# jinseokbae/neural_marionette

Measured on AMD Instinct MI355X. Metric: voxel-frames/sec (64^3, T=16), higher is better.
Workload: dtype f32 (conv products as 3x f16-split MFMA with f32 accumulate, fp32-equivalent; everything else f32); 1 GPU; AIST++-shaped synthetic clips 64^3 T=16 B=4/GPU, full NeuralMarionette.forward (detector + 11 losses + HSVRNNBVH.encode, best-of-10), fp32, random-init weights; grid=64, T=16, clips_per_gpu=4, global_clips=4, conv_mode=split16, parallelism=clip-sharded x1 (no data-path collective)

## Files before the change

### neural_marionette_amd/csrc/nm_api.hip

```cpp
#include "nm_ctx.h"
#include <mutex>
#include "nm_grad.h"
#include "nm_up2c.h"
#include <cstdarg>
#include <cstdio>
#include <cstring>
#include <cstdlib>
#include <cmath>
#include <new>
#include <stdexcept>
#include <vector>

static thread_local char g_err[512] = "";

thread_local NmLaunchState* nm_tls_ls = nullptr;
static int env_int(const char* name, int dflt) { const char* e = getenv(name); return e ? atoi(e) : dflt; }
NmLaunchState::NmLaunchState()
    : supertile(env_int("NM355_SUPERTILE", 1)),
      small16(env_int("NM355_SMALL16", 1)),
      ksplit(env_int("NM355_KSPLIT", 1)),
      occ16(env_int("NM355_OCC16", 1)),
      pool16(env_int("NM355_POOL16", 1)),
      f16p2(env_int("NM355_F16P2", 1)),
      f16p(env_int("NM355_F16P", 2)),
// ... 12 lines not shown
      sparse_first(env_int("NM355_SPARSE_FIRST", 1)),
      gn_diag(env_int("NM355_GN_DIAG", 0)),
      lazy_res(env_int("NM355_LAZY_RES", 1)),
      adjust_split(env_int("NM355_ADJUST_SPLIT", 1)),
      hg_core(env_int("NM355_HG_CORE", 1)),
      clip_occ_mfma(env_int("NM355_CLIP_OCC_MFMA", 1)),
      vrnn_chain(env_int("NM355_VRNN_CHAIN", 1)),
      wgrad_k2f16(env_int("NM355_WGRAD_K2F16", 1)),
      convt_f16(env_int("NM355_CONVT_F16", 1)),
      k5_two(env_int("NM355_K5_TWO", 0)),
      clip_late(env_int("NM355_CLIP_LATE", 1)),
      gnb_u8(env_int("NM355_GNB_U8", 1)),
      adj_zwalk(env_int("NM355_ADJ_ZWALK", 1)),
      f16q2(env_int("NM355_F16Q2", 1)),
      vrnn_post_chain(env_int("NM355_VRNN_POST_CHAIN", 2))
      , f16r(env_int("NM355_F16R", 1))
      , up2_mat(env_int("NM355_UP2_MAT", 1))
      , conv_wgs(env_int("NM355_CONV_WGS", 0))
      , fast_decode(env_int("NM355_FAST_DECODE", 1))
      , up2y(env_int("NM355_UP2Y", 1))
      , up2y_march(env_int("NM355_UP2Y_MARCH", 1))
      , up2y_ypad(env_int("NM355_UP2Y_YPAD", 1))
      , up2c_shell(env_int("NM355_UP2C_SHELL", 1))
{ store16_min = env_int("NM355_STORE16_MIN", 32768); chain_spin = env_int("NM355_CHAIN_SPIN", 1 << 20); chain_backoff = env_int("NM355_CHAIN_BACKOFF", 0); chain_drop = env_int("NM355_CHAIN_DROP_WG", 0); chain_stat_delay = env_int("NM355_CHAIN_STAT_DELAY", 0);
  chain_wgpoll = env_int("NM355_CHAIN_WGPOLL", 1);
  chain_xcd_nogo = env_int("NM355_CHAIN_XCD_NOGO", 0);
  chain_xcd = env_int("NM355_CHAIN_XCD", 1); }
NmLaunchState& nm_ls() {
    static thread_local NmLaunchState outside;
    return nm_tls_ls ? *nm_tls_ls : outside;
}

void nm_set_error(const char* fmt, ...) {
    va_list ap; va_start(ap, fmt);
    vsnprintf(g_err, sizeof(g_err), fmt, ap);
    va_end(ap);
}

int nm_abi_catch(const char* fn) noexcept {
    try { throw; }
    catch (const std::bad_alloc&) { nm_set_error("%s: out of host memory (std::bad_alloc)", fn); }
    catch (const std::exception& e) { nm_set_error("%s: internal error: %s", fn, e.what()); }
    catch (...) { nm_set_error("%s: internal error (unknown C++ exception)", fn); }
    return NM_ERR_INTERNAL;
}

// ... 104 lines not shown
    if (hipMalloc(reinterpret_cast<void**>(&c->nf_flag), sizeof(unsigned)) != hipSuccess || hipMemset(c->nf_flag, 0, sizeof(unsigned)) != hipSuccess) {
        nm_set_error("ctx_create: could not allocate the status word");
        delete c;
        return NM_ERR_HIP;
    }
    if (hipHostMalloc(reinterpret_cast<void**>(&c->nf_host), 4 * sizeof(unsigned), hipHostMallocDefault) != hipSuccess) {
        nm_set_error("ctx_create: could not allocate the pinned status slots");
        delete c;
        return NM_ERR_HIP;
    }
    for (int i = 0; i < 4; ++i) c->nf_host[i] = 0;
    { const char* e = getenv("NM355_RANGE_CHECK"); c->range_check = e ? atoi(e) : 1; }
    if (acquire_side_streams(cfg->device, &c->stream2, &c->stream3, &c->side_shared) != hipSuccess ||
        hipEventCreateWithFlags(&c->ev_w[0], hipEventDisableTiming) != hipSuccess ||
        hipEventCreateWithFlags(&c->ev_w[1], hipEventDisableTiming) != hipSuccess ||
        hipEventCreateWithFlags(&c->ev_w[2], hipEventDisableTiming) != hipSuccess ||
        hipEventCreateWithFlags(&c->ev_dy, hipEventDisableTiming) != hipSuccess ||
        hipEventCreateWithFlags(&c->ev_wjoin, hipEventDisableTiming) != hipSuccess ||
        hipEventCreateWithFlags(&c->ev_k5, hipEventDisableTiming) != hipSuccess ||
        hipEventCreateWithFlags(&c->ev_fork, hipEventDisableTiming) != hipSuccess ||
        hipEventCreateWithFlags(&c->ev_clip, hipEventDisableTiming) != hipSuccess ||
        hipEventCreateWithFlags(&c->ev_kp, hipEventDisableTiming) != hipSuccess ||
        hipEventCreateWithFlags(&c->ev_side, hipEventDisableTiming) != hipSuccess ||
        hipEventCreateWithFlags(&c->ev_nf[0], hipEventDisableTiming) != hipSuccess ||
        hipEventCreateWithFlags(&c->ev_nf[1], hipEventDisableTiming) != hipSuccess ||
        hipEventCreateWithFlags(&c->ev_nf[2], hipEventDisableTiming) != hipSuccess ||
        hipEventCreateWithFlags(&c->ev_nf[3], hipEventDisableTiming) != hipSuccess) {
        nm_set_error("ctx_create: could not create the side stream / events");
        if (c->stream2 || c->stream3) release_side_streams(cfg->device, c->stream2, c->stream3, c->side_shared);
        delete c;
        return NM_ERR_HIP;
    }
    *out = c;
    return NM_OK;
} catch (...) { return nm_abi_catch("nm_ctx_create"); }

int nm_ctx_destroy(nm_ctx* ctx) try {
    if (!ctx) return NM_OK;
    (void)hipSetDevice(ctx->cfg.device);
    (void)hipDeviceSynchronize();
    for (void* p : ctx->owned) (void)hipFree(p);
    if (ctx->ws.base) (void)hipFree(ctx->ws.base);
    if (ctx->ws2.base) (void)hipFree(ctx->ws2.base);
    if (ctx->ws_t.base) (void)hipFree(ctx->ws_t.base);
    if (ctx->copy_table) (void)hipFree(ctx->copy_table);
    if (ctx->pack_table) (void)hipFree(ctx->pack_table);
    if (ctx->nf_flag) (void)hipFree(ctx->nf_flag);
    if (ctx->nf_host) (void)hipHostFree(ctx->nf_host);
    for (hipEvent_t e : ctx->ev_nf) if (e) (void)hipEventDestroy(e);
    if (ctx->vrnn.parents) (void)hipFree(ctx->vrnn.parents);
    nm_vrnn_free_graphs(ctx);
    nm_net_free_tape(ctx);
    nm_vrnn_free_tape(ctx);
    if (ctx->stream2 || ctx->stream3) release_side_streams(ctx->cfg.device, ctx->stream2, ctx->stream3, ctx->side_shared);
    if (ctx->wside) (void)hipFree(ctx->wside);
    for (hipEvent_t e : {ctx->ev_fork, ctx->ev_clip, ctx->ev_kp, ctx->ev_side, ctx->ev_w[0], ctx->ev_w[1], ctx->ev_w[2], ctx->ev_dy, ctx->ev_wjoin, ctx->ev_k5}) if (e) (void)hipEventDestroy(e);
    for (const NmProfRec& r : ctx->ls.prof) { (void)hipEventDestroy(r.a); (void)hipEventDestroy(r.b); }
    for (hipEvent_t e : ctx->ls.event_pool) (void)hipEventDestroy(e);
    delete ctx;
    return NM_OK;
} catch (...) { return nm_abi_catch("nm_ctx_destroy"); }

int nm_ctx_set_stream(nm_ctx* ctx, void* hip_stream) try { NmScope nm_scope_(ctx);
    if (!ctx) { nm_set_error("set_stream: null ctx"); return NM_ERR_ARG; }
    hipStream_t ns = static_cast<hipStream_t>(hip_stream);
    if (ns != ctx->stream && ctx->stream_bound) {
        (void)hipSetDevice(ctx->cfg.device);
        int rc = nm_check_hip(hipEventRecord(ctx->ev_fork, ctx->stream), "set_stream: record on the old stream");
        if (!rc) rc = nm_check_hip(hipStreamWaitEvent(ns, ctx->ev_fork, 0), "set_stream: new stream waits for the old one");
        if (!rc) rc = nm_check_hip(hipEventRecord(ctx->ev_fork, ctx->stream2), "set_stream: record on the side stream");
        if (!rc) rc = nm_check_hip(hipStreamWaitEvent(ns, ctx->ev_fork, 0), "set_stream: new stream waits for the side stream");
        if (rc) return rc;
    }
    ctx->stream = ns;
    ctx->stream_bound = true;
    return NM_OK;
} catch (...) { return nm_abi_catch("nm_ctx_set_stream"); }

int nm_ctx_check_nonfinite(nm_ctx* ctx) try { NmScope nm_scope_(ctx);
// ... 358 lines not shown
```

### neural_marionette_amd/csrc/nm_common.h

```cpp
#pragma once
#include <hip/hip_runtime.h>
#include <stdint.h>
#include <vector>

#define NM_OK 0
#define NM_ERR_ARG (-1)
#define NM_ERR_HIP (-2)
#define NM_ERR_STATE (-3)
#define NM_ERR_UNSUPPORTED (-4)
#define NM_ERR_RANGE (-5)
#define NM_ERR_INTERNAL (-6)

typedef float f32x4 __attribute__((ext_vector_type(4)));
typedef float f32x16 __attribute__((ext_vector_type(16)));
typedef _Float16 nm_half8 __attribute__((ext_vector_type(8)));
template <bool SINGLE>
__device__ __forceinline__ f32x16 nm_mfma_lo(nm_half8 a, nm_half8 b, f32x16 c) {
    if constexpr (SINGLE) return c;
    else return __builtin_amdgcn_mfma_f32_32x32x16_f16(a, b, c, 0, 0, 0);
}


typedef unsigned nm_u32x2 __attribute__((ext_vector_type(2)));
typedef __bf16 nm_bf16x2 __attribute__((ext_vector_type(2)));
// ... 93 lines not shown
    if (e != hipSuccess) return nm_check_hip(e, what);
    once.mark();
    return NM_OK;
}
int nm_num_cus();
int nm_abi_catch(const char* fn) noexcept;

struct NmProfRec { hipEvent_t a, b; int variant; double flops; };
struct NmLaunchState {
    int conv_mode = 1;
    bool f16p_all = false;
    bool single = false;
    bool store16 = false;
    int op_in_h = 0, op_out_h = 0;
    int store16_min = 32768;
    int chain_spin = 1 << 20, chain_backoff = 0, chain_drop = 0, chain_fits = -1, post_chain_fits = -1, chain_stat_delay = 0, chain_wgpoll = 1, chain_xcd_nogo = 0, chain_xcd = 1, chain_cus = 0;
    bool prof_on = false;
    hipStream_t prof_stream = nullptr;
    bool prof_all = false;
    double prof_min_flops = 0.0;
    std::vector<NmProfRec> prof;
    std::vector<hipEvent_t> event_pool;
    unsigned* nf_flag = nullptr;
    int supertile, small16, ksplit, occ16, pool16, f16p2, f16p, pool_q, occ_flags, gnb_apply4, defer_sums, wgrad_async, wgrad_wgs, wgrad_tr, tail_rank1, up2c, vrnn_mid, vrnn_gemm, vrnn_graph, sparse_first, gn_diag, lazy_res, adjust_split, hg_core, clip_occ_mfma, vrnn_chain, wgrad_k2f16, convt_f16, k5_two, clip_late, gnb_u8, adj_zwalk, f16q2, vrnn_post_chain, f16r, up2_mat, conv_wgs, fast_decode, up2y, up2y_march, up2y_ypad, up2c_shell;
    NmLaunchState();
};
NmLaunchState& nm_ls();

size_t nm_packed_weight_floats(int ks, int Cin_pad, int Co_pad);
int nm_launch_pack_conv_weight(const float* w_oidhw, int Cout, int Cin, int ks, float* packed,
                               int Cin_pad, int Co_pad, hipStream_t s);
int nm_conv_blocks_per_frame(const ConvGeom& g, int Cin = 16 );
int nm_launch_conv(const TensorRef& in, const float* w_packed, const float* bias, float* out,
                   const ConvGeom& g, float* part , hipStream_t s,
                   int cin_real = 0 ,
                   const void* w_packed16 = nullptr ,
                   int out_h = 0 );
void nm_conv_set_mode(int mode);
int nm_conv_get_mode();
int nm_conv_single();
int nm_launch_pack_conv_weight16(const float* w_oidhw, int Cout, int Cin, int ks, void* packed, int Co_pad, hipStream_t s);
struct NmPackJob {
    const float* src; float* wp; void* wp16;
    int Cout, Cin, ks, Cin_pad, Co_pad, src_cin, flip, blk0, nblk;
    int src_rows;
};
int nm_pack_job_blocks(const NmPackJob& j);
int nm_launch_pack_jobs(const NmPackJob* device_jobs, int njobs, int total_blocks, hipStream_t s);
int nm_occ_blocks_per_frame(int G);
int nm_launch_pack_occ_weight(const float* w_oidhw, int Cout, float* tmp, float* packed, int Co_pad, hipStream_t s);
int nm_launch_conv_k5occ(const float* occ, int N, int G, const float* w_packed, const float* field, float* out, int Cout,
                         int Co_pad, float* part, hipStream_t s, unsigned char* brickmap = nullptr, const float* field_part = nullptr,
                         unsigned char* flags = nullptr ,
                         int out_h = 0 );
bool nm_conv_pool16_eligible(int Cin, int OD, int OH, int OW, bool have_w16);
void nm_conv_prof_enable(int on, hipStream_t stream);
int nm_conv_prof_collect(int variant, double* ms_total, double* flops_total, long long* launches);
void nm_conv_prof_reset();
struct NmProfScope {
    bool on = false; NmProfRec rec{}; hipStream_t s = nullptr;
// ... 27 lines not shown
```

### neural_marionette_amd/csrc/nm_conv.hip

```cpp
#include "nm_common.h"
#include "nm_up2c.h"
#include <type_traits>
#include <utility>
#include <vector>

namespace {

#define NM_SPLIT_SCALE 2048.0f

struct ConvParams {
    const float* in; const float* in_scale; const float* in_shift; float in_slope;
    int N, ID, IH, IW, Cin;
    const float* w; const float* bias;
    float* out; float* part;
    int OD, OH, OW, Cout, Co_pad;
    int ks, stride, pad;
    int bz_l2, by_l2, bx_l2;
    int nbz, nby, nbx;
    int KC;
    int cin_real;
    int up2;
    int HZ, HY, HX, HV, HVp;
    int CVp;
    int ZP;
// ... 2991 lines not shown
    const int io = (p.in_h ? 1 : 0) | (p.out_h ? 2 : 0);
    if (io && (!SINGLE || p.Cin > 128 || p.in2 || p.in_map || !(io & 1))) return io16_unsupported("conv_pool_f16q", p);
    NmProfScope prof(s, conv_flops(p, 8.0), 8);
    if (io) {
        if constexpr (SINGLE) {
            if (io == 3) hipLaunchKernelGGL((conv_pool_f16q_kernel<NT, true, false, 3>), grid, dim3(256), 0, s, p);
            else hipLaunchKernelGGL((conv_pool_f16q_kernel<NT, true, false, 1>), grid, dim3(256), 0, s, p);
        }
    } else
    if (nm_ls().pool_q && p.Cin <= 128) {
        if (p.in2) hipLaunchKernelGGL((conv_pool_f16q_kernel<NT, SINGLE, true>), grid, dim3(256), 0, s, p);
        else hipLaunchKernelGGL((conv_pool_f16q_kernel<NT, SINGLE, false>), grid, dim3(256), 0, s, p);
    } else
    hipLaunchKernelGGL((conv_pool_f16s_kernel<NT, SINGLE>), grid, dim3(256), 0, s, p);
    return nm_check_hip(hipGetLastError(), "conv_pool_f16s launch");
}
template <int NT>
int launch_pool_f16s(const ConvParams& p, dim3 grid, hipStream_t s) {
    return nm_ls().single ? launch_pool_f16s_impl<NT, true>(p, grid, s) : launch_pool_f16s_impl<NT, false>(p, grid, s);
}

template <auto KERNEL>
int launch_persistent(const char* what_attr, const char* what_launch, int variant, bool super_tile, const ConvParams& p_in,
                      size_t lds_bytes, int work_items, hipStream_t s) {
    static NmDeviceOnce attr_set;
    if (int rc = nm_raise_lds_limit(attr_set, 160 * 1024, what_attr, KERNEL)) return rc;
    const int cus = nm_num_cus();
    if (!cus) return NM_ERR_HIP;
    ConvParams p = p_in;
    dim3 grid((unsigned)min(work_items, nm_ls().conv_wgs > 0 ? min(nm_ls().conv_wgs, cus) : cus));
    if (super_tile) choose_super_tile(p, (int)grid.x, p.OD / 4, p.OH / 8, p.OW / 8);
    NmProfScope prof(s, conv_flops(p, 27.0), variant);
    hipLaunchKernelGGL(KERNEL, grid, dim3(512), lds_bytes, s, p);
    return nm_check_hip(hipGetLastError(), what_launch);
}

template <bool SINGLE, int IO = 0>
int launch_f16p_impl(const ConvParams& p, int work_items, hipStream_t s) {
    const size_t lds_bytes = (size_t)8 * 600 * 16 + (size_t)3 * 9 * 4 * 32 * 16 + (size_t)(256 + p.Cout) * sizeof(float);
    return launch_persistent<&conv_f16p_kernel<SINGLE, IO>>("hipFuncSetAttribute(conv_f16p)", "conv_f16p launch", 7, p.Cout == 32, p, lds_bytes, work_items, s);
}
int launch_f16p(const ConvParams& p, int work_items, hipStream_t s) {
    const int io = (p.in_h ? 1 : 0) | (p.out_h ? 2 : 0);
    if (io) {
        if (io != 3 || !nm_ls().single) return io16_unsupported("conv_f16p", p);
        return launch_f16p_impl<true, 3>(p, work_items, s);
    }
    return nm_ls().single ? launch_f16p_impl<true>(p, work_items, s) : launch_f16p_impl<false>(p, work_items, s);
}

template <bool SINGLE, int IO = 0>
int launch_f16p2_impl(const ConvParams& p, int work_items, hipStream_t s) {
    const size_t lds_bytes = (size_t)8 * 600 * 16 + (size_t)2 * 9 * 4 * 64 * 16 + (size_t)(512 + p.Cout) * sizeof(float);
    return launch_persistent<&conv_f16p2_kernel<SINGLE, IO>>("hipFuncSetAttribute(conv_f16p2)", "conv_f16p2 launch", 9, p.Cout == 64, p, lds_bytes, work_items, s);
}
template <int IO>
int launch_f16q2_impl(const ConvParams& p, int work_items, hipStream_t s) {
    const size_t lds_bytes = (size_t)4 * 600 * 16 + (size_t)2 * 27 * 2 * 64 * 16 + (size_t)(512 + p.Cout) * sizeof(float);
    if (lds_bytes > 160 * 1024) { nm_set_error("conv_f16q2: %d output channels exceed the LDS budget", p.Cout); return NM_ERR_UNSUPPORTED; }
    return launch_persistent<&conv_f16q2_kernel<IO>>("hipFuncSetAttribute(conv_f16q2)", "conv_f16q2 launch", 14, p.Cout == 64, p, lds_bytes, work_items, s);
}
template <int IO, int C16T>
int launch_f16r_impl(const ConvParams& p, int work_items, hipStream_t s) {
    const size_t lds_bytes = (size_t)4 * 600 * 16 + (size_t)27 * C16T * 64 * 16 + (size_t)(512 + 32) * sizeof(float) + 2048 + 256 + 1024;
    return launch_persistent<&conv_f16r_kernel<IO, C16T>>("hipFuncSetAttribute(conv_f16r)", "conv_f16r launch", 15, true, p, lds_bytes, work_items, s);
}
int launch_f16p2(const ConvParams& p, int work_items, hipStream_t s) {
    const int io = (p.in_h ? 1 : 0) | (p.out_h ? 2 : 0);
    if (nm_ls().single && nm_ls().f16q2 && (io == 0 || io == 3) && p.Cout <= 1024) {
        return io ? launch_f16q2_impl<3>(p, work_items, s) : launch_f16q2_impl<0>(p, work_items, s);
    }
    if (io) {
        if (io != 3 || !nm_ls().single) return io16_unsupported("conv_f16p2", p);
        return launch_f16p2_impl<true, 3>(p, work_items, s);
    }
    if (nm_ls().single) return launch_f16p2_impl<true>(p, work_items, s);
    return launch_f16p2_impl<false>(p, work_items, s);
}

#ifdef NM_DIAG
unsigned long long* g_stamps = nullptr;
#endif

}

#ifdef NM_DIAG
extern "C" void nm_diag_set_stamps(void* p) { g_stamps = static_cast<unsigned long long*>(p); }
#endif
void nm_conv_set_mode(int mode) { NmLaunchState& l = nm_ls(); l.conv_mode = mode ? 1 : 0; l.f16p_all = mode == 2; l.single = mode == 3 || mode == 4; l.store16 = mode == 4; }
int nm_conv_get_mode() { const NmLaunchState& l = nm_ls(); return l.conv_mode && l.single ? (l.store16 ? 4 : 3) : (l.conv_mode && l.f16p_all ? 2 : l.conv_mode); }
int nm_conv_single() { return nm_ls().conv_mode && nm_ls().single; }

int nm_launch_pack_conv_weight16(const float* w, int Cout, int Cin, int ks, void* packed, int Co_pad, hipStream_t s) {
    if (Co_pad % 32 || Cout > Co_pad) { nm_set_error("pack_conv_weight16: bad padding Cout=%d/%d", Cout, Co_pad); return NM_ERR_ARG; }
    size_t total = (size_t)ks * ks * ks * ((Cin + 15) / 16) * 2 * Co_pad * 8;
    int blocks = (int)min((total + 255) / 256, (size_t)2048);
    hipLaunchKernelGGL(pack_conv_weight16_kernel, dim3(blocks), dim3(256), 0, s, w, Cout, Cin, ks, reinterpret_cast<_Float16*>(packed), Co_pad);
    return nm_check_hip(hipGetLastError(), "pack_conv_weight16 launch");
}

// ... 106 lines not shown
NmProfScope::~NmProfScope() {
    if (!on) return;
    (void)hipEventRecord(rec.b, s);
    nm_ls().prof.push_back(rec);
}

int nm_num_cus() {
    static int cus = 0;
    if (cus == 0) {
        int dev = 0; hipDeviceProp_t prop;
        if (hipGetDevice(&dev) != hipSuccess || hipGetDeviceProperties(&prop, dev) != hipSuccess) { (void)nm_check_hip(hipErrorUnknown, "device query"); return 0; }
        cus = prop.multiProcessorCount > 0 ? prop.multiProcessorCount : 256;
    }
    return cus;
}

void nm_conv_prof_reset() {
    NmLaunchState& l = nm_ls();
    for (const NmProfRec& r : l.prof) { l.event_pool.push_back(r.a); l.event_pool.push_back(r.b); }
    l.prof.clear();
}

int nm_launch_conv(const TensorRef& in, const float* w_packed, const float* bias, float* out,
                   const ConvGeom& g, float* part, hipStream_t s, int cin_real, const void* w_packed16, int out_h) {
    if (in.C % 8 != 0 || g.Co_pad % 32 != 0 || g.Cout > g.Co_pad || g.Cout <= 0) {
        nm_set_error("conv: unsupported channels Cin=%d Cout=%d Co_pad=%d", in.C, g.Cout, g.Co_pad);
        return NM_ERR_ARG;
    }
    const int us = g.up2 ? 2 : 1;
    if ((us * in.D + 2 * g.pad - g.ks) / g.stride + 1 != g.OD || (us * in.H + 2 * g.pad - g.ks) / g.stride + 1 != g.OH ||
        (us * in.W + 2 * g.pad - g.ks) / g.stride + 1 != g.OW) {
        nm_set_error("conv: geometry mismatch in=(%d,%d,%d) k=%d s=%d p=%d out=(%d,%d,%d)", in.D, in.H, in.W,
                     g.ks, g.stride, g.pad, g.OD, g.OH, g.OW);
        return NM_ERR_ARG;
    }
    if ((in.scale == nullptr) != (in.shift == nullptr)) { nm_set_error("conv: scale/shift must come together"); return NM_ERR_ARG; }
    if ((in.brickmap || in.p2) && g.up2) { nm_set_error("conv: a brick-sparse input tensor can only feed the k2 s2 split-fp16 pool kernel"); return NM_ERR_ARG; }
    if (use_up2c(g, in.C)) {
        double flops = 2.0 * in.N * (double)g.OD * g.OH * g.OW * g.Cout * (double)(cin_real > 0 ? cin_real : in.C) * 27.0;
        if (nm_up2y_active()) flops *= 0.5;
        NmProfScope prof(s, flops, 12);
        return nm_launch_conv_up2c(in, g.up2c, bias, out, g.Cout, g.Co_pad, part, s, out_h);
    }
    Tiling t = choose_tiling(g, in.C);
    if (t.lds_bytes > 160 * 1024) { nm_set_error("conv: LDS tile %zu B too large", t.lds_bytes); return NM_ERR_UNSUPPORTED; }
    ConvParams p;
    p.in = in.p; p.in_scale = in.scale; p.in_shift = in.shift; p.in_slope = in.slope;
// ... 19 lines not shown
    p.w16 = (nm_ls().conv_mode == 1 && nm_ls().small16 && w_packed16 && in.C % 8 == 0 && !g.up2 && t.MT == 1 && (t.KC % 16 == 0 || t.KC == in.C)) ? w_packed16 : nullptr;
    if (p.w16) t.lds_bytes = max(t.lds_bytes, (size_t)(((t.KC + 15) & ~15) / 4) * (t.HVp + t.CVp) * 16);
    p.ksplit = 1;
    if (p.w16 && nm_ls().ksplit) {
        const int top = ((min(g.OD, 1 << t.bz_l2) - 1) << (t.bx_l2 + t.by_l2)) + ((min(g.OH, 1 << t.by_l2) - 1) << t.bx_l2) + min(g.OW, 1 << t.bx_l2) - 1;
        const int rw = top / 32 + 1;
        p.ksplit = rw == 1 ? 4 : (rw == 2 ? 2 : 1);
        if (p.ksplit > 1) t.lds_bytes = max(t.lds_bytes, (size_t)4 * t.NT * 16 * 64 * sizeof(float));
    }
#ifdef NM_DIAG
    p.stamps = g_stamps;
#endif
    p.KC = t.KC; p.HZ = t.HZ; p.HY = t.HY; p.HX = t.HX; p.HV = t.HV; p.HVp = t.HVp; p.CVp = t.CVp; p.ZP = t.HY * t.HX;
    dim3 grid((unsigned)(in.N * t.nbz * t.nby * t.nbx), (unsigned)(g.Co_pad / (t.NT * 32)));
    if (pool16_case(t, in.C, w_packed16 != nullptr) && g.ks == 2 && g.stride == 2 && g.pad == 0 && !g.up2) {
        p.w = static_cast<const float*>(w_packed16);
        return t.NT == 2 ? launch_pool_f16s<2>(p, grid, s) : launch_pool_f16s<1>(p, grid, s);
    }
    const bool k3_bricks = w_packed16 && in.C % 16 == 0 && g.ks == 3 && g.stride == 1 && g.pad == 1 && !g.up2 &&
                           g.OD % 4 == 0 && g.OH % 8 == 0 && g.OW % 8 == 0 && g.OD >= 16;
    if (nm_ls().conv_mode == 1 && nm_ls().f16p2 && k3_bricks && g.Cout % 64 == 0) {
        const int work = in.N * (g.OD / 4) * (g.OH / 8) * (g.OW / 8) * (g.Cout / 64);
        p.w = static_cast<const float*>(w_packed16);
        return launch_f16p2(p, work, s);
    }
    if (nm_ls().conv_mode == 1 && nm_ls().single && nm_ls().f16r && nm_ls().f16p && k3_bricks && (in.C == 32 || in.C == 64) && g.Cout == 32 &&
        (p.in_h != 0) == (p.out_h != 0)) {
        const int work = in.N * (g.OD / 4) * (g.OH / 8) * (g.OW / 8);
        p.w = static_cast<const float*>(w_packed16);
        if (in.C == 32) return p.in_h ? launch_f16r_impl<3, 2>(p, work, s) : launch_f16r_impl<0, 2>(p, work, s);
        return p.in_h ? launch_f16r_impl<3, 4>(p, work, s) : launch_f16r_impl<0, 4>(p, work, s);
    }
    if (nm_ls().conv_mode == 1 && nm_ls().f16p && k3_bricks && g.Cout % 32 == 0 && (nm_ls().f16p == 1 || nm_ls().f16p_all || g.Cout == 32)) {
        const int work = in.N * (g.OD / 4) * (g.OH / 8) * (g.OW / 8) * (g.Cout / 32);
        p.w = static_cast<const float*>(w_packed16);
        return launch_f16p(p, work, s);
    }
    if (nm_ls().conv_mode == 1 && w_packed16 && in.C % 16 == 0 && t.MT == 2 && t.bx_l2 == 3 && t.by_l2 == 3 && t.bz_l2 == 2 &&
        g.stride == 1 && (g.ks == 1 || g.ks == 3) && t.HZ == g.ks + 3 && t.HY * t.HX * 2 <= 256) {
        Tiling t16 = t;
        const int area = t.HY * t.HX;
        p.ZP = area + ((4 - (area & 15)) & 15);
        const int hv = t.HZ * p.ZP;
        p.HVp = hv + ((2 - (hv & 7)) & 7);
        const bool blds = (t.NT == 1 && g.ks == 3);
        const size_t bbytes = blds ? (size_t)2 * 9 * 4 * 32 * 16 : 0;
        t16.lds_bytes = max(blds ? (size_t)4 * p.HVp * 16 + bbytes : (size_t)4 * (p.HVp + t.CVp) * 16, (size_t)4 * 64 * 2 * sizeof(float));
        if (t16.lds_bytes <= 80 * 1024) {
            p.w = static_cast<const float*>(w_packed16);
            if (g.ks == 3 && g.up2) return t.NT == 2 ? launch_f16s<2, 2, 3, true>(p, t16, grid, s) : launch_f16s<2, 1, 3, true>(p, t16, grid, s);
            if (g.ks == 3) return t.NT == 2 ? launch_f16s<2, 2, 3, false>(p, t16, grid, s) : launch_f16s<2, 1, 3, false>(p, t16, grid, s);
            if (!g.up2) return t.NT == 2 ? launch_f16s<2, 2, 1, false>(p, t16, grid, s) : launch_f16s<2, 1, 1, false>(p, t16, grid, s);
        }
        p.HVp = t.HVp;
    }
    if (p.in_h || p.out_h) return io16_unsupported("conv (fp32 MFMA kernel)", p);
    if (t.MT == 2 && t.NT == 2) return launch_t<2, 2>(p, t, grid, s);
    if (t.MT == 2 && t.NT == 1) return launch_t<2, 1>(p, t, grid, s);
    if (t.MT == 1 && t.NT == 2) return launch_t<1, 2>(p, t, grid, s);
// ... 49 lines not shown
```

### neural_marionette_amd/csrc/nm_ctx.h

```cpp
#pragma once
#include "nm_common.h"
#include "../../include/nm355.h"
#include <map>
#include <string>
#include <vector>

struct Arena {
    char* base = nullptr;
    size_t cap = 0, top = 0, peak = 0;
    bool dry = false;
    bool overflow = false;

    void* alloc_bytes(size_t bytes) {
        size_t a = (top + 255) & ~(size_t)255;
        top = a + bytes;
        if (top > peak) peak = top;
        if (dry) return reinterpret_cast<void*>((uintptr_t)256);
        if (top > cap) { overflow = true; return nullptr; }
        return base + a;
    }
    float* f(size_t n) { return static_cast<float*>(alloc_bytes(n * sizeof(float))); }
    size_t mark() const { return top; }
    void release(size_t m) { top = m; }
};
// ... 42 lines not shown

struct VrnnW {
    LinearW post0, post2, prior0, prior2, root0, root2, joint0, joint2;
    float *w_ih = nullptr, *w_hh = nullptr, *b_ih = nullptr, *b_hh = nullptr;
    float* h0 = nullptr;
    float* offset_param = nullptr;
    int32_t* parents = nullptr;
    int32_t* order = nullptr;
    int32_t* lvl_joint = nullptr;
    int32_t* lvl_start = nullptr;
    int nlevels = 0;
    std::vector<int32_t> parents_h, order_h;
    bool has_tree = false;
    uint64_t tree_epoch = 0;
};

struct nm_ctx {
    nm_config cfg;
    NmLaunchState ls;
    hipStream_t stream = nullptr;
    bool stream_bound = false;
    hipStream_t stream2 = nullptr;
    hipEvent_t ev_fork = nullptr, ev_clip = nullptr, ev_kp = nullptr, ev_side = nullptr;
    hipStream_t stream3 = nullptr;
    bool side_shared = false;
    hipEvent_t ev_w[3] = {nullptr, nullptr, nullptr}, ev_dy = nullptr, ev_wjoin = nullptr, ev_k5 = nullptr;
    float* wside = nullptr; size_t wside_floats = 0;
    size_t wside_slot = 0, wside_scratch = 0, wside_sc = 0;
    hipEvent_t ev_user_decoder = nullptr;
    unsigned* nf_flag = nullptr;
    unsigned* nf_host = nullptr;
    hipEvent_t ev_nf[4] = {nullptr, nullptr, nullptr, nullptr};
    bool nf_busy[4] = {false, false, false, false};
    uint64_t nf_seq[4] = {0, 0, 0, 0};
    const char* nf_who[4] = {nullptr, nullptr, nullptr, nullptr};
    uint64_t nf_calls = 0;
    unsigned nf_last = 0;
    int range_check = 1;
    int learn_sigma = 0;
    int gauss_cat = 0;
    int affinity_ver = 3;
    int graph_loss_ver = 1;
    int const_intensity = 3;
    int graph_flags = 0;
    bool graph_none() const { return (graph_flags & NM_GRAPH_NONE) != 0; }
    int64_t affinity_numel() const {
// ... 45 lines not shown
```

### neural_marionette_amd/csrc/nm_net.hip

```cpp
#include "nm_ctx.h"
#include "nm_heads.h"
#include "nm_grad.h"
#include "nm_heads_bwd.h"
#include "nm_up2c.h"
#include "nm_hgcore.h"
#include <cmath>
#include <cstdio>
#include <vector>
#include <algorithm>
#include <functional>

struct ConvRec {
    const ConvW* w = nullptr; const NormW* gn = nullptr;
    TensorRef in{}, out{};
    TensorRef upmat{};
    const float* fpart = nullptr; int nblk = 0;
    const double* chsum = nullptr;
    int stride = 1, pad = 0; bool up2 = false;
};
struct ResRec { ConvRec c1, c2, cs; bool has_skip = false; };
struct UpRec { const UpW* w = nullptr; TensorRef in{}, out{}; const float* fpart = nullptr; int nblk = 0; const double* chsum = nullptr; };
struct HgRec { ResRec s1, e1, s2, e2, s3, e3, d3, d2, d1; ConvRec p1, p2, p3; UpRec u3, u2, u1; };
struct FeatRec {
    const FeatNetW* w = nullptr; const float* occ = nullptr; int N = 0, G = 0;
// ... 228 lines not shown
        if (!r && !c->training && nm_conv_get_mode() == 1 && nm_ls().occ16 && nm_ls().sparse_first) {
            const int nblk = nm_occ_blocks_per_frame(G);
            f.field_part = nm_ctx_weight_alloc(c, (size_t)nblk * Cout * 2);
            float* scratch = nm_ctx_weight_alloc(c, G3 * Cout);
            if (!f.field_part || !scratch) r = NM_ERR_HIP;
            else r = nm_launch_conv_k5occ(zero, 1, G, f.occ_w, f.field, scratch, Cout, f.c0.Co_pad, f.field_part, c->stream);
        }
        if (r && !rc) rc = r;
    }
    LinearW linear(const std::string& p, int out, int in) {
        LinearW l; l.in = in; l.out = out; l.w = copy(p + ".weight", (int64_t)out * in); l.b = copy(p + ".bias", out); return l;
    }
};

__global__ void pack_small_kernel(const float* a, int na, const float* b, int nb, float* out) {
    int i = threadIdx.x;
    if (i < na) out[i] = a[i];
    else if (i < na + nb) out[i] = b[i - na];
}

struct Net {
    nm_ctx* c; hipStream_t s; Arena& ws; int rc = NM_OK;
    bool keep = false;
    explicit Net(nm_ctx* ctx) : c(ctx), s(ctx->stream), ws(ctx->ws) {}
    Net(nm_ctx* ctx, hipStream_t stream) : c(ctx), s(stream), ws(ctx->ws) {}
    void release(size_t m) { if (!keep) ws.release(m); }
    bool ok() const { return rc == NM_OK; }
    bool live() const { return rc == NM_OK && !ws.dry; }
    void run(int r) { if (r && !rc) rc = r; }
    float* alloc(size_t n) {
        float* p = ws.f(n);
        if (!p && !rc) { nm_set_error("workspace overflow (needed > %zu bytes)", ws.cap); rc = NM_ERR_STATE; }
        return p;
    }
    int h16(size_t voxels_per_frame) const { return keep && nm_ls().store16 && voxels_per_frame >= (size_t)nm_ls().store16_min ? 1 : 0; }
    float* alloc_e(size_t elems, int h) { return alloc(h ? (elems + 1) / 2 : elems); }
};

TensorRef mk(const float* p, int N, int D, int H, int W, int C, const float* sc = nullptr, const float* sh = nullptr, float slope = 1.0f) {
    TensorRef t; t.p = p; t.scale = sc; t.shift = sh; t.slope = slope; t.N = N; t.D = D; t.H = H; t.W = W; t.C = C; return t;
}
TensorRef with_h(TensorRef t, int h) { t.h = h; return t; }
size_t vox(const TensorRef& t) { return (size_t)t.D * t.H * t.W; }

TensorRef conv_gn(Net& n, const TensorRef& in, const ConvW& w, const NormW* gn, int stride, int pad, float slope_after,
                  float* out_buf = nullptr, bool up2 = false, ConvRec* rec = nullptr) {
    ConvGeom g; g.ks = w.ks; g.stride = stride; g.pad = pad; g.up2 = up2 ? 1 : 0;
    const int us = up2 ? 2 : 1;
    g.OD = (us * in.D + 2 * pad - w.ks) / stride + 1; g.OH = (us * in.H + 2 * pad - w.ks) / stride + 1; g.OW = (us * in.W + 2 * pad - w.ks) / stride + 1;
// ... 1 lines not shown
    const size_t ov = (size_t)g.OD * g.OH * g.OW;
    const int oh = out_buf ? 0 : n.h16(ov);
    TensorRef src = in;
    const bool mat = up2 && rec && n.keep && !out_buf && nm_ls().single && nm_ls().up2_mat && nm_ls().f16r && w.wp16 && w.ks == 3 && stride == 1 && pad == 1 &&
                     w.Cout == 32 && (in.C == 32 || in.C == 64) && g.OD % 4 == 0 && g.OH % 8 == 0 && g.OW % 8 == 0 && g.OD >= 16;
    if (mat) {
        float* upb = n.alloc_e((size_t)in.N * ov * in.C, oh);
        if (n.live()) n.run(nm_launch_upsample2(in, upb, n.s, oh));
        src = with_h(mk(upb, in.N, g.OD, g.OH, g.OW, in.C), oh);
        g.up2 = 0; g.up2c = nullptr;
    }
    float* out = out_buf ? out_buf : n.alloc_e((size_t)in.N * ov * w.Cout, oh);
    float *part = nullptr, *scale = nullptr, *shift = nullptr;
    const int nblk = nm_conv_blocks_per_frame(g, in.C);
    double* chsum = nullptr;
    if (gn) {
        part = n.alloc((size_t)in.N * nblk * w.Cout * 2);
        scale = n.alloc((size_t)in.N * w.Cout); shift = n.alloc((size_t)in.N * w.Cout);
        if (rec && nm_gn_finalize_has_chsum(w.Cout, gn->groups)) chsum = reinterpret_cast<double*>(n.alloc((size_t)in.N * w.Cout * 4));
    }
    if (n.live()) {
        if (in.C != w.Cin_pad) { nm_set_error("conv_gn: input has %d channels, layer expects %d", in.C, w.Cin_pad); n.rc = NM_ERR_STATE; }
        else {
            n.run(nm_launch_conv(src, w.wp, w.bias, out, g, part, n.s, w.Cin, w.wp16, oh));
            if (gn) n.run(nm_launch_gn_finalize(part, in.N, nblk, w.Cout, gn->groups, (double)ov * (w.Cout / gn->groups),
                                                gn->gamma, gn->beta, 1e-5f, scale, shift, n.s, chsum));
            if (gn && nm_ls().gn_diag && !oh) n.run(nm_launch_gn_direct(out, in.N, (int)ov, w.Cout, gn->groups, gn->gamma, gn->beta, 1e-5f, scale, shift, n.s, chsum));
        }
    }
    TensorRef o = with_h(mk(out, in.N, g.OD, g.OH, g.OW, w.Cout, scale, shift, slope_after), oh);
    if (rec) { rec->w = &w; rec->gn = gn; rec->in = in; rec->out = o; rec->fpart = part; rec->nblk = nblk; rec->chsum = chsum; rec->stride = stride; rec->pad = pad; rec->up2 = up2; rec->upmat = mat ? src : TensorRef{}; }
    return o;
}

TensorRef add2(Net& n, const TensorRef& a, const TensorRef* b, float* out_buf = nullptr) {
    const int oh = out_buf ? 0 : n.h16(vox(a));
    float* out = out_buf ? out_buf : n.alloc_e((size_t)a.N * vox(a) * a.C, oh);
    if (n.live()) n.run(nm_launch_apply2(a, b, out, n.s, oh));
    return with_h(mk(out, a.N, a.D, a.H, a.W, a.C), oh);
}

TensorRef res(Net& n, const TensorRef& x, const ResW& w, float* out_buf = nullptr, ResRec* rec = nullptr, bool lazy_sum = false) {
    if (lazy_sum && !rec && !out_buf) {
        TensorRef r1 = conv_gn(n, x, w.c1, &w.n1, 1, 1, LRELU);
        TensorRef r2 = conv_gn(n, r1, w.c2, &w.n2, 1, 1, 1.0f);
        TensorRef sk = w.has_skip ? conv_gn(n, x, w.cs, &w.ns, 1, 0, 1.0f) : x;
        TensorRef o = r2;
// ... 74 lines not shown
        if (!n.rc) {
            if (nm_conv_get_mode() != 1) nm_set_error("hourglass core: conv mode %d (the fused launch is split-fp16 arithmetic: mode 1 only)", nm_conv_get_mode());
            else if (a2.D < 2 || a2.D > 6) nm_set_error("hourglass core: level-2 extent %d (the fused launch takes 2 .. 6)", a2.D);
            else if (nm_hg_core_scratch_items(hp) < 0) nm_set_error("hourglass core: %zu bytes of LDS per frame do not fit", nm_hg_core_lds_bytes(hp));
            else nm_set_error("hourglass core: a layer has no split-fp16 weight pack (or the channel counts do not chain)");
            n.rc = NM_ERR_UNSUPPORTED;
        }
        return a2;
    }
    if (eligible) {
        float* d2out = n.alloc((size_t)a2.N * vox(a2) * w.d2.c2.Cout);
        hp.out = d2out;
        if (n.live()) n.run(nm_launch_hg_core(hp, n.s));
        return mk(d2out, a2.N, a2.D, a2.H, a2.W, w.d2.c2.Cout);
    }
    TensorRef x = res(n, a2, w.e2, nullptr, r ? &r->e2 : nullptr);
    TensorRef s3 = res(n, x, w.s3, nullptr, r ? &r->s3 : nullptr);
    x = res(n, pool(n, x, w.p3, r ? &r->p3 : nullptr), w.e3, nullptr, r ? &r->e3 : nullptr);
    x = res(n, x, w.d3, nullptr, r ? &r->d3 : nullptr);
    TensorRef u = up(n, x, w.u3, op3, r ? &r->u3 : nullptr); x = add2(n, u, &s3);
    return res(n, x, w.d2, nullptr, r ? &r->d2 : nullptr);
}

TensorRef hourglass(Net& n, const TensorRef& x0, const HourglassW& w, int Ng, HgRec* r = nullptr) {
    const int op3 = (Ng / 4) % 2, op2 = (Ng / 2) % 2, op1 = Ng % 2;
    TensorRef s1 = res(n, x0, w.s1, nullptr, r ? &r->s1 : nullptr);
    TensorRef x = res(n, pool(n, x0, w.p1, r ? &r->p1 : nullptr), w.e1, nullptr, r ? &r->e1 : nullptr);
    TensorRef s2 = res(n, x, w.s2, nullptr, r ? &r->s2 : nullptr);
    TensorRef a2 = pool(n, x, w.p2, r ? &r->p2 : nullptr);
    x = hourglass_core(n, a2, w, op3, r);
    TensorRef u = up(n, x, w.u2, op2, r ? &r->u2 : nullptr); x = add2(n, u, &s2);
    x = res(n, x, w.d1, nullptr, r ? &r->d1 : nullptr);
    u = up(n, x, w.u1, op1, r ? &r->u1 : nullptr); x = add2(n, u, &s1);
    return x;
}

TensorRef first_layer(Net& n, const float* occ, int N, int G, const FeatNetW& w, FeatRec* rec = nullptr) {
    const int Cout = w.c0.Cout;
    const size_t G3 = (size_t)G * G * G;
    const int oh = rec ? n.h16(G3) : 0;
    float* out = n.alloc_e((size_t)N * G3 * Cout, oh);
    const int nblk = nm_occ_blocks_per_frame(G);
    float* part = n.alloc((size_t)N * nblk * Cout * 2);
    const bool sparse = !rec && w.field_part && nm_conv_get_mode() == 1 && nm_ls().occ16 && nm_ls().sparse_first &&
                        nm_conv_pool16_eligible(Cout, G / 2, G / 2, G / 2, w.p1.c.wp16 != nullptr);
    unsigned char* bmap = sparse ? reinterpret_cast<unsigned char*>(n.alloc(((size_t)N * nblk + 3) / 4)) : nullptr;
    unsigned char* bflags = sparse ? reinterpret_cast<unsigned char*>(n.alloc(((size_t)N * nblk + 3) / 4)) : nullptr;
    float* scale = n.alloc((size_t)N * Cout); float* shift = n.alloc((size_t)N * Cout);
    double* chsum = (rec && nm_gn_finalize_has_chsum(Cout, w.n0.groups)) ? reinterpret_cast<double*>(n.alloc((size_t)N * Cout * 4)) : nullptr;
    if (n.live()) {
        n.run(nm_launch_conv_k5occ(occ, N, G, w.occ_w, w.field, out, Cout, w.c0.Co_pad, part, n.s, bmap, sparse ? w.field_part : nullptr, bflags, oh));
        n.run(nm_launch_gn_finalize(part, N, nblk, Cout, w.n0.groups, (double)G3 * (Cout / w.n0.groups), w.n0.gamma, w.n0.beta,
                                    1e-5f, scale, shift, n.s, chsum));
        if (nm_ls().gn_diag && !sparse && !oh) n.run(nm_launch_gn_direct(out, N, (int)G3, Cout, w.n0.groups, w.n0.gamma, w.n0.beta, 1e-5f, scale, shift, n.s, chsum));
    }
    TensorRef o = with_h(mk(out, N, G, G, G, Cout, scale, shift, LRELU), oh);
// ... 59 lines not shown
                                         Cc, comb, n.s, c->gauss_cat));
            x = mk(comb, nf, g, g, g, Cc);
            x = conv_gn(n, x, d.adjust, nullptr, 1, 0, LRELU, nullptr, false, tape ? &tape->adjust : nullptr);
        }
        x = conv_gn(n, x, d.d1, &d.dn2, 1, 1, LRELU, nullptr, true, tape ? &tape->d1 : nullptr);
        x = conv_gn(n, x, d.d4, &d.dn5, 1, 1, LRELU, nullptr, false, tape ? &tape->d4 : nullptr);
        x = conv_gn(n, x, d.d8, &d.dn9, 1, 1, LRELU, nullptr, true, tape ? &tape->d8 : nullptr);
        x = conv_gn(n, x, d.d11, &d.dn12, 1, 1, LRELU, nullptr, false, tape ? &tape->d11 : nullptr);
        if (n.live())
            n.run(nm_launch_decoder_tail(x, d.d14, first_frames + (size_t)b0 * ff_stride * G3, ff_stride, T,
                                         target ? target + (size_t)f0 * G3 : nullptr,
                                         (target && chamfer) ? keypoints + (size_t)f0 * K * 4 : nullptr, K, G,
                                         recon + (size_t)f0 * G3, tail_part ? tail_part + (size_t)f0 * tb * 3 : nullptr, n.s));
        n.release(m1);
    }
    n.release(m0);
}

int detector_graph(nm_ctx* c, const float* vox_in, int B, int T, int affinity_on, float* keypoints, float* heatmaps,
                   float* first_feature, float* recon, float* affinity, float* losses,
                   const std::function<int()>* after_keypoints = nullptr, TrainTape* tape = nullptr) {
    Net n(c);
    n.keep = tape != nullptr;
    const DetectorW& d = c->det;
    if (c->graph_none()) affinity_on = 0;
    const int K = c->cfg.nkeypoints, G = c->cfg.grid_size, g = G / 4, F = B * T, N = c->cfg.nneighbor;
    const size_t g3 = (size_t)g * g * g, G3 = (size_t)G * G * G;
    const int Kc = d.head.Cout;
    n.ws.release(0);
    float* feat = n.alloc((size_t)F * g3 * FEAT);
    float* clip_head = n.alloc((size_t)B * g3 * Kc);
    float* heat_part = n.alloc((size_t)F * K * g * (2 * g + 2));
    float* heat_mean = n.alloc((size_t)F * K);
    float* clip_part = n.alloc((size_t)B * 5);
    const int tb = nm_tail_blocks(G);
    float* tail_part = n.alloc((size_t)F * tb * 3);
    float* frame_sums = n.alloc((size_t)F * 3);
    float* aff = affinity_on ? (affinity ? affinity : n.alloc((size_t)N * K * K)) : nullptr;

    auto clip_block = [&]() {
        Net n2(c, c->stream2);
        n2.keep = n.keep;
        float* in = n2.alloc((size_t)B * G3);
        float* fclip = n2.alloc((size_t)B * g3 * 2 * FEAT);
        if (n2.live()) n2.run(nm_launch_mean_t(vox_in, B, T, G3, in, n2.s));
        feature_net(n2, in, B, G, d.clip, g, fclip, tape ? &tape->clip : nullptr);
// ... 944 lines not shown
```

Before: 3976 voxel-frames/s.

## Run hourglass skip-branch residual on a side stream with capped conv workgroups

Result: faster. 4044 voxel-frames/s, median of 6 (+1.7%).

```diff
diff --git a/neural_marionette_amd/csrc/nm_api.hip b/neural_marionette_amd/csrc/nm_api.hip
--- a/neural_marionette_amd/csrc/nm_api.hip
+++ b/neural_marionette_amd/csrc/nm_api.hip
@@ -58,6 +58,9 @@
       , up2y_march(env_int("NM355_UP2Y_MARCH", 1))
       , up2y_ypad(env_int("NM355_UP2Y_YPAD", 1))
       , up2c_shell(env_int("NM355_UP2C_SHELL", 1))
+      , enc_sched(env_int("NM355_ENC_SCHED", 1))
+      , enc_s1(env_int("NM355_ENC_S1", 1))
+      , enc_s1_wgs(env_int("NM355_ENC_S1_WGS", -1))
 { store16_min = env_int("NM355_STORE16_MIN", 32768); chain_spin = env_int("NM355_CHAIN_SPIN", 1 << 20); chain_backoff = env_int("NM355_CHAIN_BACKOFF", 0); chain_drop = env_int("NM355_CHAIN_DROP_WG", 0); chain_stat_delay = env_int("NM355_CHAIN_STAT_DELAY", 0);
   chain_wgpoll = env_int("NM355_CHAIN_WGPOLL", 1);
   chain_xcd_nogo = env_int("NM355_CHAIN_XCD_NOGO", 0);
@@ -208,6 +211,8 @@
         hipEventCreateWithFlags(&c->ev_clip, hipEventDisableTiming) != hipSuccess ||
         hipEventCreateWithFlags(&c->ev_kp, hipEventDisableTiming) != hipSuccess ||
         hipEventCreateWithFlags(&c->ev_side, hipEventDisableTiming) != hipSuccess ||
+        hipEventCreateWithFlags(&c->ev_s1_fork, hipEventDisableTiming) != hipSuccess ||
+        hipEventCreateWithFlags(&c->ev_s1_join, hipEventDisableTiming) != hipSuccess ||
         hipEventCreateWithFlags(&c->ev_nf[0], hipEventDisableTiming) != hipSuccess ||
         hipEventCreateWithFlags(&c->ev_nf[1], hipEventDisableTiming) != hipSuccess ||
         hipEventCreateWithFlags(&c->ev_nf[2], hipEventDisableTiming) != hipSuccess ||
@@ -240,7 +245,7 @@
     nm_vrnn_free_tape(ctx);
     if (ctx->stream2 || ctx->stream3) release_side_streams(ctx->cfg.device, ctx->stream2, ctx->stream3, ctx->side_shared);
     if (ctx->wside) (void)hipFree(ctx->wside);
-    for (hipEvent_t e : {ctx->ev_fork, ctx->ev_clip, ctx->ev_kp, ctx->ev_side, ctx->ev_w[0], ctx->ev_w[1], ctx->ev_w[2], ctx->ev_dy, ctx->ev_wjoin, ctx->ev_k5}) if (e) (void)hipEventDestroy(e);
+    for (hipEvent_t e : {ctx->ev_fork, ctx->ev_clip, ctx->ev_kp, ctx->ev_side, ctx->ev_s1_fork, ctx->ev_s1_join, ctx->ev_w[0], ctx->ev_w[1], ctx->ev_w[2], ctx->ev_dy, ctx->ev_wjoin, ctx->ev_k5}) if (e) (void)hipEventDestroy(e);
     for (const NmProfRec& r : ctx->ls.prof) { (void)hipEventDestroy(r.a); (void)hipEventDestroy(r.b); }
     for (hipEvent_t e : ctx->ls.event_pool) (void)hipEventDestroy(e);
     delete ctx;
diff --git a/neural_marionette_amd/csrc/nm_common.h b/neural_marionette_amd/csrc/nm_common.h
--- a/neural_marionette_amd/csrc/nm_common.h
+++ b/neural_marionette_amd/csrc/nm_common.h
@@ -139,7 +139,7 @@
     std::vector<NmProfRec> prof;
     std::vector<hipEvent_t> event_pool;
     unsigned* nf_flag = nullptr;
-    int supertile, small16, ksplit, occ16, pool16, f16p2, f16p, pool_q, occ_flags, gnb_apply4, defer_sums, wgrad_async, wgrad_wgs, wgrad_tr, tail_rank1, up2c, vrnn_mid, vrnn_gemm, vrnn_graph, sparse_first, gn_diag, lazy_res, adjust_split, hg_core, clip_occ_mfma, vrnn_chain, wgrad_k2f16, convt_f16, k5_two, clip_late, gnb_u8, adj_zwalk, f16q2, vrnn_post_chain, f16r, up2_mat, conv_wgs, fast_decode, up2y, up2y_march, up2y_ypad, up2c_shell;
+    int supertile, small16, ksplit, occ16, pool16, f16p2, f16p, pool_q, occ_flags, gnb_apply4, defer_sums, wgrad_async, wgrad_wgs, wgrad_tr, tail_rank1, up2c, vrnn_mid, vrnn_gemm, vrnn_graph, sparse_first, gn_diag, lazy_res, adjust_split, hg_core, clip_occ_mfma, vrnn_chain, wgrad_k2f16, convt_f16, k5_two, clip_late, gnb_u8, adj_zwalk, f16q2, vrnn_post_chain, f16r, up2_mat, conv_wgs, fast_decode, up2y, up2y_march, up2y_ypad, up2c_shell, enc_sched, enc_s1, enc_s1_wgs;
     NmLaunchState();
 };
 NmLaunchState& nm_ls();
@@ -152,7 +152,8 @@
                    const ConvGeom& g, float* part , hipStream_t s,
                    int cin_real = 0 ,
                    const void* w_packed16 = nullptr ,
-                   int out_h = 0 );
+                   int out_h = 0 ,
+                   int wgs_cap = 0 );
 void nm_conv_set_mode(int mode);
 int nm_conv_get_mode();
 int nm_conv_single();
diff --git a/neural_marionette_amd/csrc/nm_conv.hip b/neural_marionette_amd/csrc/nm_conv.hip
--- a/neural_marionette_amd/csrc/nm_conv.hip
+++ b/neural_marionette_amd/csrc/nm_conv.hip
@@ -3037,13 +3037,15 @@
 
 template <auto KERNEL>
 int launch_persistent(const char* what_attr, const char* what_launch, int variant, bool super_tile, const ConvParams& p_in,
-                      size_t lds_bytes, int work_items, hipStream_t s) {
+                      size_t lds_bytes, int work_items, hipStream_t s, int wgs_cap) {
     static NmDeviceOnce attr_set;
     if (int rc = nm_raise_lds_limit(attr_set, 160 * 1024, what_attr, KERNEL)) return rc;
     const int cus = nm_num_cus();
     if (!cus) return NM_ERR_HIP;
     ConvParams p = p_in;
-    dim3 grid((unsigned)min(work_items, nm_ls().conv_wgs > 0 ? min(nm_ls().conv_wgs, cus) : cus));
+    int wgs = nm_ls().conv_wgs > 0 ? min(nm_ls().conv_wgs, cus) : cus;
+    if (wgs_cap > 0 && wgs_cap < wgs) wgs = min(wgs, max(8, wgs_cap & ~7));
+    dim3 grid((unsigned)min(work_items, wgs));
     if (super_tile) choose_super_tile(p, (int)grid.x, p.OD / 4, p.OH / 8, p.OW / 8);
     NmProfScope prof(s, conv_flops(p, 27.0), variant);
     hipLaunchKernelGGL(KERNEL, grid, dim3(512), lds_bytes, s, p);
@@ -3051,46 +3053,46 @@
 }
 
 template <bool SINGLE, int IO = 0>
-int launch_f16p_impl(const ConvParams& p, int work_items, hipStream_t s) {
+int launch_f16p_impl(const ConvParams& p, int work_items, hipStream_t s, int wgs_cap) {
     const size_t lds_bytes = (size_t)8 * 600 * 16 + (size_t)3 * 9 * 4 * 32 * 16 + (size_t)(256 + p.Cout) * sizeof(float);
-    return launch_persistent<&conv_f16p_kernel<SINGLE, IO>>("hipFuncSetAttribute(conv_f16p)", "conv_f16p launch", 7, p.Cout == 32, p, lds_bytes, work_items, s);
-}
-int launch_f16p(const ConvParams& p, int work_items, hipStream_t s) {
+    return launch_persistent<&conv_f16p_kernel<SINGLE, IO>>("hipFuncSetAttribute(conv_f16p)", "conv_f16p launch", 7, p.Cout == 32, p, lds_bytes, work_items, s, wgs_cap);
+}
+int launch_f16p(const ConvParams& p, int work_items, hipStream_t s, int wgs_cap) {
     const int io = (p.in_h ? 1 : 0) | (p.out_h ? 2 : 0);
     if (io) {
         if (io != 3 || !nm_ls().single) return io16_unsupported("conv_f16p", p);
-        return launch_f16p_impl<true, 3>(p, work_items, s);
-    }
-    return nm_ls().single ? launch_f16p_impl<true>(p, work_items, s) : launch_f16p_impl<false>(p, work_items, s);
+        return launch_f16p_impl<true, 3>(p, work_items, s, wgs_cap);
+    }
+    return nm_ls().single ? launch_f16p_impl<true>(p, work_items, s, wgs_cap) : launch_f16p_impl<false>(p, work_items, s, wgs_cap);
 }
 
 template <bool SINGLE, int IO = 0>
-int launch_f16p2_impl(const ConvParams& p, int work_items, hipStream_t s) {
+int launch_f16p2_impl(const ConvParams& p, int work_items, hipStream_t s, int wgs_cap) {
     const size_t lds_bytes = (size_t)8 * 600 * 16 + (size_t)2 * 9 * 4 * 64 * 16 + (size_t)(512 + p.Cout) * sizeof(float);
-    return launch_persistent<&conv_f16p2_kernel<SINGLE, IO>>("hipFuncSetAttribute(conv_f16p2)", "conv_f16p2 launch", 9, p.Cout == 64, p, lds_bytes, work_items, s);
+    return launch_persistent<&conv_f16p2_kernel<SINGLE, IO>>("hipFuncSetAttribute(conv_f16p2)", "conv_f16p2 launch", 9, p.Cout == 64, p, lds_bytes, work_items, s, wgs_cap);
 }
 template <int IO>
-int launch_f16q2_impl(const ConvParams& p, int work_items, hipStream_t s) {
+int launch_f16q2_impl(const ConvParams& p, int work_items, hipStream_t s, int wgs_cap) {
     const size_t lds_bytes = (size_t)4 * 600 * 16 + (size_t)2 * 27 * 2 * 64 * 16 + (size_t)(512 + p.Cout) * sizeof(float);
     if (lds_bytes > 160 * 1024) { nm_set_error("conv_f16q2: %d output channels exceed the LDS budget", p.Cout); return NM_ERR_UNSUPPORTED; }
-    return launch_persistent<&conv_f16q2_kernel<IO>>("hipFuncSetAttribute(conv_f16q2)", "conv_f16q2 launch", 14, p.Cout == 64, p, lds_bytes, work_items, s);
+    return launch_persistent<&conv_f16q2_kernel<IO>>("hipFuncSetAttribute(conv_f16q2)", "conv_f16q2 launch", 14, p.Cout == 64, p, lds_bytes, work_items, s, wgs_cap);
 }
 template <int IO, int C16T>
-int launch_f16r_impl(const ConvParams& p, int work_items, hipStream_t s) {
+int launch_f16r_impl(const ConvParams& p, int work_items, hipStream_t s, int wgs_cap) {
     const size_t lds_bytes = (size_t)4 * 600 * 16 + (size_t)27 * C16T * 64 * 16 + (size_t)(512 + 32) * sizeof(float) + 2048 + 256 + 1024;
-    return launch_persistent<&conv_f16r_kernel<IO, C16T>>("hipFuncSetAttribute(conv_f16r)", "conv_f16r launch", 15, true, p, lds_bytes, work_items, s);
-}
-int launch_f16p2(const ConvParams& p, int work_items, hipStream_t s) {
+    return launch_persistent<&conv_f16r_kernel<IO, C16T>>("hipFuncSetAttribute(conv_f16r)", "conv_f16r launch", 15, true, p, lds_bytes, work_items, s, wgs_cap);
+}
+int launch_f16p2(const ConvParams& p, int work_items, hipStream_t s, int wgs_cap) {
     const int io = (p.in_h ? 1 : 0) | (p.out_h ? 2 : 0);
     if (nm_ls().single && nm_ls().f16q2 && (io == 0 || io == 3) && p.Cout <= 1024) {
-        return io ? launch_f16q2_impl<3>(p, work_items, s) : launch_f16q2_impl<0>(p, work_items, s);
+        return io ? launch_f16q2_impl<3>(p, work_items, s, wgs_cap) : launch_f16q2_impl<0>(p, work_items, s, wgs_cap);
     }
     if (io) {
         if (io != 3 || !nm_ls().single) return io16_unsupported("conv_f16p2", p);
-        return launch_f16p2_impl<true, 3>(p, work_items, s);
-    }
-    if (nm_ls().single) return launch_f16p2_impl<true>(p, work_items, s);
-    return launch_f16p2_impl<false>(p, work_items, s);
+        return launch_f16p2_impl<true, 3>(p, work_items, s, wgs_cap);
+    }
+    if (nm_ls().single) return launch_f16p2_impl<true>(p, work_items, s, wgs_cap);
+    return launch_f16p2_impl<false>(p, work_items, s, wgs_cap);
 }
 
 #ifdef NM_DIAG
@@ -3243,7 +3245,7 @@
 }
 
 int nm_launch_conv(const TensorRef& in, const float* w_packed, const float* bias, float* out,
-                   const ConvGeom& g, float* part, hipStream_t s, int cin_real, const void* w_packed16, int out_h) {
+                   const ConvGeom& g, float* part, hipStream_t s, int cin_real, const void* w_packed16, int out_h, int wgs_cap) {
     if (in.C % 8 != 0 || g.Co_pad % 32 != 0 || g.Cout > g.Co_pad || g.Cout <= 0) {
         nm_set_error("conv: unsupported channels Cin=%d Cout=%d Co_pad=%d", in.C, g.Cout, g.Co_pad);
         return NM_ERR_ARG;
@@ -3309,19 +3311,19 @@
     if (nm_ls().conv_mode == 1 && nm_ls().f16p2 && k3_bricks && g.Cout % 64 == 0) {
         const int work = in.N * (g.OD / 4) * (g.OH / 8) * (g.OW / 8) * (g.Cout / 64);
         p.w = static_cast<const float*>(w_packed16);
-        return launch_f16p2(p, work, s);
+        return launch_f16p2(p, work, s, wgs_cap);
     }
     if (nm_ls().conv_mode == 1 && nm_ls().single && nm_ls().f16r && nm_ls().f16p && k3_bricks && (in.C == 32 || in.C == 64) && g.Cout == 32 &&
         (p.in_h != 0) == (p.out_h != 0)) {
         const int work = in.N * (g.OD / 4) * (g.OH / 8) * (g.OW / 8);
         p.w = static_cast<const float*>(w_packed16);
-        if (in.C == 32) return p.in_h ? launch_f16r_impl<3, 2>(p, work, s) : launch_f16r_impl<0, 2>(p, work, s);
-        return p.in_h ? launch_f16r_impl<3, 4>(p, work, s) : launch_f16r_impl<0, 4>(p, work, s);
+        if (in.C == 32) return p.in_h ? launch_f16r_impl<3, 2>(p, work, s, wgs_cap) : launch_f16r_impl<0, 2>(p, work, s, wgs_cap);
+        return p.in_h ? launch_f16r_impl<3, 4>(p, work, s, wgs_cap) : launch_f16r_impl<0, 4>(p, work, s, wgs_cap);
     }
     if (nm_ls().conv_mode == 1 && nm_ls().f16p && k3_bricks && g.Cout % 32 == 0 && (nm_ls().f16p == 1 || nm_ls().f16p_all || g.Cout == 32)) {
         const int work = in.N * (g.OD / 4) * (g.OH / 8) * (g.OW / 8) * (g.Cout / 32);
         p.w = static_cast<const float*>(w_packed16);
-        return launch_f16p(p, work, s);
+        return launch_f16p(p, work, s, wgs_cap);
     }
     if (nm_ls().conv_mode == 1 && w_packed16 && in.C % 16 == 0 && t.MT == 2 && t.bx_l2 == 3 && t.by_l2 == 3 && t.bz_l2 == 2 &&
         g.stride == 1 && (g.ks == 1 || g.ks == 3) && t.HZ == g.ks + 3 && t.HY * t.HX * 2 <= 256) {
diff --git a/neural_marionette_amd/csrc/nm_ctx.h b/neural_marionette_amd/csrc/nm_ctx.h
--- a/neural_marionette_amd/csrc/nm_ctx.h
+++ b/neural_marionette_amd/csrc/nm_ctx.h
@@ -88,6 +88,7 @@
     bool stream_bound = false;
     hipStream_t stream2 = nullptr;
     hipEvent_t ev_fork = nullptr, ev_clip = nullptr, ev_kp = nullptr, ev_side = nullptr;
+    hipEvent_t ev_s1_fork = nullptr, ev_s1_join = nullptr;
     hipStream_t stream3 = nullptr;
     bool side_shared = false;
     hipEvent_t ev_w[3] = {nullptr, nullptr, nullptr}, ev_dy = nullptr, ev_wjoin = nullptr, ev_k5 = nullptr;
diff --git a/neural_marionette_amd/csrc/nm_net.hip b/neural_marionette_amd/csrc/nm_net.hip
--- a/neural_marionette_amd/csrc/nm_net.hip
+++ b/neural_marionette_amd/csrc/nm_net.hip
@@ -274,9 +274,12 @@
 struct Net {
     nm_ctx* c; hipStream_t s; Arena& ws; int rc = NM_OK;
     bool keep = false;
+    int conv_wgs = 0;
+    bool s1_fork = false;
+    bool hold = false;
     explicit Net(nm_ctx* ctx) : c(ctx), s(ctx->stream), ws(ctx->ws) {}
     Net(nm_ctx* ctx, hipStream_t stream) : c(ctx), s(stream), ws(ctx->ws) {}
-    void release(size_t m) { if (!keep) ws.release(m); }
+    void release(size_t m) { if (!keep && !hold) ws.release(m); }
     bool ok() const { return rc == NM_OK; }
     bool live() const { return rc == NM_OK && !ws.dry; }
     void run(int r) { if (r && !rc) rc = r; }
@@ -324,7 +327,7 @@
     if (n.live()) {
         if (in.C != w.Cin_pad) { nm_set_error("conv_gn: input has %d channels, layer expects %d", in.C, w.Cin_pad); n.rc = NM_ERR_STATE; }
         else {
-            n.run(nm_launch_conv(src, w.wp, w.bias, out, g, part, n.s, w.Cin, w.wp16, oh));
+            n.run(nm_launch_conv(src, w.wp, w.bias, out, g, part, n.s, w.Cin, w.wp16, oh, n.conv_wgs));
             if (gn) n.run(nm_launch_gn_finalize(part, in.N, nblk, w.Cout, gn->groups, (double)ov * (w.Cout / gn->groups),
                                                 gn->gamma, gn->beta, 1e-5f, scale, shift, n.s, chsum));
             if (gn && nm_ls().gn_diag && !oh) n.run(nm_launch_gn_direct(out, in.N, (int)ov, w.Cout, gn->groups, gn->gamma, gn->beta, 1e-5f, scale, shift, n.s, chsum));
@@ -445,16 +448,40 @@
     return res(n, x, w.d2, nullptr, r ? &r->d2 : nullptr);
 }
 
+static TensorRef res_on_stream3(Net& n, const TensorRef& x, const ResW& w, hipEvent_t ev_fork, hipEvent_t ev_join, int wgs_cap, bool& forked) {
+    nm_ctx* c = n.c;
+    Net n3(c, c->stream3);
+    n3.hold = true; n3.rc = n.rc; n3.conv_wgs = wgs_cap;
+    forked = false;
+    if (n.live()) {
+        n.run(nm_check_hip(hipEventRecord(ev_fork, n.s), "hourglass: skip-branch fork event"));
+        n.run(nm_check_hip(hipStreamWaitEvent(c->stream3, ev_fork, 0), "hourglass: skip-branch stream wait"));
+        n3.rc = n.rc; forked = n.ok();
+    }
+    TensorRef o = res(n3, x, w);
+    if (forked) n.run(nm_check_hip(hipEventRecord(ev_join, c->stream3), "hourglass: skip-branch join event"));
+    n.run(n3.rc);
+    return o;
+}
+
 TensorRef hourglass(Net& n, const TensorRef& x0, const HourglassW& w, int Ng, HgRec* r = nullptr) {
     const int op3 = (Ng / 4) % 2, op2 = (Ng / 2) % 2, op1 = Ng % 2;
-    TensorRef s1 = res(n, x0, w.s1, nullptr, r ? &r->s1 : nullptr);
+    nm_ctx* c = n.c;
+    const bool fork = n.s1_fork && !r && c->stream3 && c->stream3 != n.s;
+    bool forked1 = false;
+    int cap = nm_ls().enc_s1_wgs;
+    if (fork && cap < 0) { const int cus = nm_num_cus(); cap = cus > 16 ? std::max(cus / 2, cus - 2 * x0.N) : 0; }
+    TensorRef s1 = fork ? res_on_stream3(n, x0, w.s1, c->ev_s1_fork, c->ev_s1_join, cap, forked1)
+                        : res(n, x0, w.s1, nullptr, r ? &r->s1 : nullptr);
     TensorRef x = res(n, pool(n, x0, w.p1, r ? &r->p1 : nullptr), w.e1, nullptr, r ? &r->e1 : nullptr);
     TensorRef s2 = res(n, x, w.s2, nullptr, r ? &r->s2 : nullptr);
     TensorRef a2 = pool(n, x, w.p2, r ? &r->p2 : nullptr);
     x = hourglass_core(n, a2, w, op3, r);
     TensorRef u = up(n, x, w.u2, op2, r ? &r->u2 : nullptr); x = add2(n, u, &s2);
     x = res(n, x, w.d1, nullptr, r ? &r->d1 : nullptr);
-    u = up(n, x, w.u1, op1, r ? &r->u1 : nullptr); x = add2(n, u, &s1);
+    u = up(n, x, w.u1, op1, r ? &r->u1 : nullptr);
+    if (forked1) n.run(nm_check_hip(hipStreamWaitEvent(n.s, c->ev_s1_join, 0), "hourglass: join the skip branch"));
+    x = add2(n, u, &s1);
     return x;
 }
 
@@ -560,6 +587,7 @@
                    const std::function<int()>* after_keypoints = nullptr, TrainTape* tape = nullptr) {
     Net n(c);
     n.keep = tape != nullptr;
+    n.s1_fork = !tape && nm_ls().enc_sched && nm_ls().enc_s1;
     const DetectorW& d = c->det;
     if (c->graph_none()) affinity_on = 0;
     const int K = c->cfg.nkeypoints, G = c->cfg.grid_size, g = G / 4, F = B * T, N = c->cfg.nneighbor;
```
